# imagemagick/ImageMagick

Measured on NVIDIA H100. Metric: Mpixels/s on 8K RGBA Gaussian-blur σ=4 + Lanczos 2×; % HBM roofline, higher is better.
Workload: dtype f64

## Files before the change

imagemagick_b200/build.py:

```python
from __future__ import annotations

import os
import shutil
import subprocess
import sys
from concurrent.futures import ThreadPoolExecutor
from pathlib import Path

PKG = Path(__file__).resolve().parent
ROOT = PKG.parent
CSRC = PKG / "csrc"
LIBDIR = PKG / "lib"
OBJDIR = LIBDIR / "obj"
LIB = LIBDIR / "libmagickb200.so"

ARCH = ["-gencode", "arch=compute_90a,code=sm_90a"]
NVCC_FLAGS = ["-O3", "-std=c++17", "-lineinfo", "-Xcompiler", "-fPIC,-fvisibility=hidden,-ffp-contract=off",
              "-Xptxas", "-v"]

SOURCES = ["runtime.cu", "kernel_info.cpp", "resize_filter.cpp", "resize_tables.cpp", "conv1d.cu", "conv_mma.cu",
           "morph2d.cu", "morph_stream.cu", "morph_direct.cu", "cache.cu", "resize.cu", "resize_stream.cu", "colorspace.cu", "hexcone.cu", "pointwise.cu", "equalize.cu", "stencils.cu", "hooks.cu", "enhance.cu", "layout.cu", "level.cu",
           "distort_plan.cpp", "distort.cu", "geometry_plan.cpp", "geometry.cu", "api.cu"]
FILE_FLAGS = {"distort.cu": ["-fmad=false"]}


def _nvcc() -> str:
    for cand in (os.environ.get("NVCC"), shutil.which("nvcc"), "/usr/local/cuda/bin/nvcc"):
        if cand and Path(cand).exists():
            return cand
    raise RuntimeError("nvcc not found; libmagickb200 cannot be built")


def _stale(target: Path, deps: list[Path]) -> bool:
    if not target.exists():
        return True
    t = target.stat().st_mtime
    return any(d.stat().st_mtime > t for d in deps if d.exists())


def build(force: bool = False, verbose: bool = False) -> Path:
    nvcc = _nvcc()
    OBJDIR.mkdir(parents=True, exist_ok=True)
    headers = list(CSRC.glob("*.h")) + list(CSRC.glob("*.cuh")) + list((ROOT / "include").glob("*.h"))
    jobs = []
    for name in SOURCES:
        src = CSRC / name
        obj = OBJDIR / (src.stem + ".o")
        if force or _stale(obj, [src] + headers):
            cmd = [nvcc, *ARCH, *NVCC_FLAGS, *FILE_FLAGS.get(name, []), "-x", "cu", "-c", str(src), "-o", str(obj)]
            jobs.append((name, cmd, obj))

    def run(job):
        name, cmd, obj = job
        p = subprocess.run(cmd, capture_output=True, text=True)
# ... 27 lines not shown
```

imagemagick_b200/csrc/api.cu:

```cuda
#include "mb200_internal.h"

#include <cuda_runtime.h>

#include <cmath>
#include <cstdlib>
#include <memory>
#include <vector>

using namespace mb200;

namespace {

struct StreamAlloc {
  void *ptr = nullptr;
  cudaStream_t s;
  explicit StreamAlloc(cudaStream_t stream) : s(stream) {}
  int alloc(size_t bytes) {
    cudaError_t e = cudaMallocAsync(&ptr, bytes ? bytes : 1, temp_pool(), s);
    if (e != cudaSuccess) { ptr = nullptr; return cuda_fail(e, "cudaMallocAsync"); }
    return MB200_OK;
  }
  ~StreamAlloc() { if (ptr) cudaFreeAsync(ptr, s); }
  StreamAlloc(const StreamAlloc &) = delete;
  StreamAlloc &operator=(const StreamAlloc &) = delete;
// ... 80 lines not shown
          if (rc != MB200_EUNSUPPORTED) return rc;
        }
      }
    }
  }
  if ((method == MB200_ErodeMorphology || method == MB200_DilateMorphology) && d_counter == nullptr &&
      !knobs.no_morph_stream) {
    const int rc = launch_morph_stream(src, dst, w, h, ch, method, win.data(), kw, kh, ox, oy, s);
    if (rc != MB200_EUNSUPPORTED) return rc;
  }
  double gamma_scale = 1.0;
  if (method == MB200_ConvolveMorphology && kw == 1) {
    size_t count = 0;
    for (double v : win) if (!std::isnan(v)) ++count;
    if (count != 0) gamma_scale = static_cast<double>(kh) / static_cast<double>(count);
  }
  return launch_morph2d(src, dst, w, h, ch, method, win.data(), kw, kh, ox, oy, bias, gamma_scale, d_counter, s);
}

int counted_primitive(const float *src, float *dst, size_t w, size_t h, int ch, int method, const mb200_kernel_info *k,
                      double bias, unsigned long long *d_counter, long long *changed, cudaStream_t s) {
  cudaMemsetAsync(d_counter, 0, sizeof(unsigned long long), s);
  const int rc = primitive(src, dst, w, h, ch, method, k, bias, d_counter, s);
  if (rc) return rc;
  unsigned long long hostv = 0;
  cudaError_t e = cudaMemcpyAsync(&hostv, d_counter, sizeof(hostv), cudaMemcpyDeviceToHost, s);
  if (e == cudaSuccess) e = cudaStreamSynchronize(s);
  if (e != cudaSuccess) return cuda_fail(e, "changed readback");
  *changed = static_cast<long long>(hostv / static_cast<unsigned long long>(ch));
  return MB200_OK;
}

struct Stage { int primitive; const mb200_kernel_info *kernel; };

int apply_hit_and_miss_family(const float *src, float *dst, size_t w, size_t h, int ch, int method, long iterations,
                              const mb200_kernel_info *kernel, cudaStream_t s) {
  const size_t method_limit = iterations < 0 ? (w > h ? w : h) : static_cast<size_t>(iterations);
  const bool unite = method == MB200_HitAndMissMorphology && kernel->next != nullptr;
  const size_t bytes = w * h * static_cast<size_t>(ch) * sizeof(float), npix = w * h;
  StreamAlloc a(s), b(s), united(s), counter(s);
  int rc = a.alloc(bytes);
  if (!rc) rc = b.alloc(bytes);
  if (!rc && unite) rc = united.alloc(bytes);
  if (!rc) rc = counter.alloc(sizeof(unsigned long long));
  if (rc) return rc;
  float *bufs[2] = {static_cast<float *>(a.ptr), static_cast<float *>(b.ptr)};
  unsigned long long *d_counter = static_cast<unsigned long long *>(counter.ptr);
  const float *cur = src;
  int next = 0;
  bool have_united = false;
  size_t round = 0;
  long long round_changed = 1;
  while (round < method_limit && round_changed > 0) {
    ++round;
    round_changed = 0;
    for (const mb200_kernel_info *k = kernel; k; k = k->next) {
      if (method_limit > 1) {
        long long changed = 0;
        rc = counted_primitive(cur, bufs[next], w, h, ch, method, k, 0.0, d_counter, &changed, s);
        round_changed += changed;
      } else {
        rc = primitive(cur, bufs[next], w, h, ch, method, k, 0.0, nullptr, s);
      }
      if (rc) return rc;
      cur = bufs[next];
      next ^= 1;
// ... 63 lines not shown
    rotate_kernel_info(reflected.get(), 180.0);
  }
  std::vector<Stage> stages;
  const mb200_kernel_info *rk = reflected.get();
  for (const mb200_kernel_info *nk = kernel; nk; nk = nk->next, rk = rk ? rk->next : nullptr) {
    for (int stage = 1; stage <= stage_limit; ++stage) {
      Stage st{method, nk};
      switch (method) {
        case MB200_OpenMorphology: st.primitive = stage == 2 ? MB200_DilateMorphology : MB200_ErodeMorphology; break;
        case MB200_CloseMorphology: st.kernel = rk; st.primitive = stage == 2 ? MB200_ErodeMorphology : MB200_DilateMorphology; break;
        case MB200_OpenIntensityMorphology:
          st.primitive = stage == 2 ? MB200_DilateIntensityMorphology : MB200_ErodeIntensityMorphology;
          break;
        case MB200_CloseIntensityMorphology:
          st.kernel = rk;
          st.primitive = stage == 2 ? MB200_ErodeIntensityMorphology : MB200_DilateIntensityMorphology;
          break;
        case MB200_SmoothMorphology:
          if (stage == 1) st.primitive = MB200_ErodeMorphology;
          else if (stage == 2) st.primitive = MB200_DilateMorphology;
          else if (stage == 3) { st.kernel = rk; st.primitive = MB200_DilateMorphology; }
          else { st.kernel = rk; st.primitive = MB200_ErodeMorphology; }
          break;
        case MB200_CorrelateMorphology: st.kernel = rk; st.primitive = MB200_ConvolveMorphology; break;
        default: break;
      }
      stages.push_back(st);
    }
  }
  const size_t bytes = w * h * static_cast<size_t>(ch) * sizeof(float);
  int rc = MB200_OK;
  if (kernel_limit == 1) {
    const size_t total = stages.size();
    StreamAlloc tmp(s);
    if (total > 1) { rc = tmp.alloc(bytes); }
    const float *cur = src;
    for (size_t i = 0; i < total && rc == MB200_OK; ++i) {
      float *out = ((total - 1 - i) % 2 == 0) ? dst : static_cast<float *>(tmp.ptr);
      const bool last = i + 1 == total;
      rc = primitive(cur, out, w, h, ch, stages[i].primitive, stages[i].kernel, bias, nullptr, s,
                     last ? epilogue : nullptr, last ? epilogue_fused : nullptr);
      cur = out;
    }
  } else {
    StreamAlloc a(s), b(s), counter(s);
    rc = a.alloc(bytes);
    if (!rc) rc = b.alloc(bytes);
    if (!rc) rc = counter.alloc(sizeof(unsigned long long));
    const float *cur = src;
    float *bufs[2] = {static_cast<float *>(a.ptr), static_cast<float *>(b.ptr)};
    int next = 0;
    for (size_t i = 0; i < stages.size() && rc == MB200_OK; ++i) {
      size_t loop = 0;
      long long changed = 1;
      while (loop < kernel_limit && changed > 0 && rc == MB200_OK) {
        ++loop;
        rc = counted_primitive(cur, bufs[next], w, h, ch, stages[i].primitive, stages[i].kernel, bias,
                               static_cast<unsigned long long *>(counter.ptr), &changed, s);
        cur = bufs[next];
        next ^= 1;
      }
    }
    if (rc == MB200_OK) {
      cudaError_t e = cudaMemcpyAsync(dst, cur, bytes, cudaMemcpyDeviceToDevice, s);
      if (e != cudaSuccess) rc = cuda_fail(e, "result copy");
    }
// ... 1103 lines not shown
```

imagemagick_b200/csrc/conv_common.cuh:

```cuda
#pragma once

#include <cuda_runtime.h>

namespace mb200 {
namespace {

constexpr double kQuantumScale = 1.0 / 65535.0;
constexpr double kEpsilon = 1.0e-12;

__device__ __forceinline__ bool nonfinite_bits(float v) { return (__float_as_uint(v) & 0x7f800000u) == 0x7f800000u; }
__device__ __forceinline__ bool nonfinite_bits(double v) {
  return (static_cast<unsigned>(__double2hiint(v)) & 0x7ff00000u) == 0x7ff00000u;
}

__device__ __forceinline__ double clamp_denominator(double den) {
  constexpr double kTiny = kEpsilon / kQuantumScale;
  const unsigned hi = static_cast<unsigned>(__double2hiint(den));
  const unsigned long long mag = (static_cast<unsigned long long>(hi & 0x7fffffffu) << 32) | static_cast<unsigned>(__double2loint(den));
  const unsigned long long tiny = static_cast<unsigned long long>(__double_as_longlong(kTiny));
  if (mag < tiny)
    den = __hiloint2double(static_cast<int>((hi & 0x80000000u) | static_cast<unsigned>(tiny >> 32)), static_cast<int>(tiny & 0xffffffffu));
  return den;
}

__device__ __forceinline__ float unsharp_point(float p, float blurred, double gain, double qthreshold) {
  const double d = __dsub_rn(static_cast<double>(p), static_cast<double>(blurred));
  if (fabs(__dmul_rn(2.0, d)) < qthreshold) return p;
  return static_cast<float>(__dadd_rn(static_cast<double>(p), __dmul_rn(gain, d)));
}

__device__ __forceinline__ double fast_reciprocal(double g) {
  double r0;
  asm("rcp.approx.ftz.f64 %0, %1;" : "=d"(r0) : "d"(g));
  const double e0 = fma(-g, r0, 1.0);
  const double r1 = fma(r0, e0, r0);
  const double e1 = fma(-g, r1, 1.0);
  return fma(r1, e1, r1);
}

__device__ __forceinline__ double shfl_double(double v, int lane) {
  int lo = __double2loint(v), hi = __double2hiint(v);
  lo = __shfl_sync(0xffffffffu, lo, lane);
  hi = __shfl_sync(0xffffffffu, hi, lane);
  return __hiloint2double(hi, lo);
}

}
}
```

imagemagick_b200/csrc/conv_mma.cu:

```cuda
#include "mb200_internal.h"
#include "conv_common.cuh"

#include <cuda_runtime.h>

#include <cstdint>

namespace mb200 {
namespace {

template <int NKS>
struct MmaTaps { double k[4 * NKS]; };

struct MmaArgs {
  const void *src;
  void *dst;
  int width, height;
  int off;
  int ntaps;
  int strip;
  const float *aux;
  double gain, qthreshold;
  int l2pf;
};

// ... 246 lines not shown
      ahead[0] = raw[0]; ahead[1] = raw[1];
      raw[0] = keep0; raw[1] = keep1;
    }
    output(prev, epi_prev, prev_valid);
    if (b > 0) outp += ostep;

    if (window_bad != 0) {
#pragma unroll
      for (int g = 0; g < 2; ++g) {
        double s0 = 0.0, s1 = 0.0, s2 = 0.0, s3 = 0.0;
        int u = 8 * sb + n8;
        if (u >= RR) u -= RR;
        for (int t = 0; t < a.ntaps; ++t) {
          const double *p = ring + static_cast<unsigned>(u) * kUStride + lane_px_off + g * kGroup;
          const double2 rg = *reinterpret_cast<const double2 *>(p);
          const double2 ba = *reinterpret_cast<const double2 *>(p + kBA);
          const double k = taps.k[t];
          s0 = fma(k, rg.x, s0); s1 = fma(k, rg.y, s1); s2 = fma(k, ba.x, s2); s3 = fma(k, ba.y, s3);
          if (++u == RR) u = 0;
        }
        acc[2 * g][0] = s0; acc[2 * g][1] = s1; acc[2 * g + 1][0] = s2; acc[2 * g + 1][1] = s3;
      }
    }
#pragma unroll
    for (int t = 0; t < 4; ++t) { prev[t][0] = acc[t][0]; prev[t][1] = acc[t][1]; }
    if (EPI) { epi_prev[0] = epi_cur[0]; epi_prev[1] = epi_cur[1]; }
    prev_valid = mvalid;
    st_slot = st_slot + 1 == NB ? 0 : st_slot + 1;
    if (++sb == NB) sb = 0;
  }
  output(prev, epi_prev, prev_valid);
}

template <int NKS>
struct WideTaps { double k[16 * NKS]; };

template <int NKS, int AXIS, int EPI>
__global__ void __launch_bounds__(128, 3) conv_mma_wide_kernel(const MmaArgs a, const WideTaps<NKS> taps) {
  static_assert(EPI == 0 || AXIS == 1, "the fused epilogue belongs to the final column pass");
  constexpr int NB = NKS + 1;
  constexpr int RR = 16 * NB;
  constexpr int PW = 36;
  constexpr int PL = 2 * RR + 8;
  constexpr int kWarpDoubles = AXIS == 1 ? RR * PW : 16 * PL;
  extern __shared__ __align__(16) double ring_all[];
  const int warp = threadIdx.x >> 5, lane = threadIdx.x & 31;
  double *ring = ring_all + warp * kWarpDoubles;
  const unsigned ring_s = static_cast<unsigned>(__cvta_generic_to_shared(ring));
  const int t4 = lane & 3, g8 = lane >> 2;

  int first, nout, limit, par0;
  if (AXIS == 1) {
    par0 = (blockIdx.x * 4 + warp) * 8;
    if (par0 >= a.width) return;
    first = blockIdx.y * a.strip;
    nout = min(a.strip, a.height - first);
    limit = a.height - 1;
  } else {
    par0 = (blockIdx.y * 4 + warp) * 8;
    if (par0 >= a.height) return;
    first = blockIdx.x * a.strip;
    nout = min(a.strip, a.width - first);
    limit = a.width - 1;
  }
  const int nblocks = (nout + 15) >> 4;
  const bool mma_l2pf = a.l2pf != 0;
  const size_t pitch = static_cast<size_t>(a.width) * 16;

// ... 10 lines not shown
    } else {
      const int line = lh + 4 * (i >> 1);
      lbase[i] = static_cast<const char *>(a.src) + static_cast<size_t>(min(par0 + line, a.height - 1)) * pitch;
      uoff[i] = lq + 8 * (i & 1);
      st_off[i] = static_cast<unsigned>(line * PL + 2 * uoff[i]);
    }
  }
  constexpr unsigned kBlockStride = AXIS == 1 ? 16 * PW : 32;
  constexpr unsigned kBA = AXIS == 1 ? 16 : 8 * PL;
  const size_t lstep = AXIS == 1 ? pitch : 16;
  const int base = first - a.off;

  float4 raw[4];
  auto fetch = [&](int j) {
#pragma unroll
    for (int i = 0; i < 4; ++i) {
      const unsigned pos = static_cast<unsigned>(min(max(base + 16 * j + uoff[i], 0), limit));
      raw[i] = __ldg(reinterpret_cast<const float4 *>(lbase[i] + static_cast<size_t>(pos) * lstep));
    }
  };
  constexpr int kL2Ahead = 4;
  auto prefetch_l2 = [&](int j) {
#pragma unroll
    for (int i = 0; i < 4; ++i) {
      const unsigned pos = static_cast<unsigned>(min(max(base + 16 * j + uoff[i], 0), limit));
      asm volatile("prefetch.global.L2 [%0];" ::"l"(lbase[i] + static_cast<size_t>(pos) * lstep));
    }
  };
  unsigned badmask = 0;
  auto stage = [&](int slot) {
    bool bad = false;
#pragma unroll
    for (int i = 0; i < 4; ++i) {
      const float4 f = raw[i];
      const unsigned m = max(max(__float_as_uint(f.x) & 0x7fffffffu, __float_as_uint(f.y) & 0x7fffffffu),
                             max(__float_as_uint(f.z) & 0x7fffffffu, __float_as_uint(f.w) & 0x7fffffffu));
      bad = bad || m >= 0x7f800000u;
      const double da = static_cast<double>(f.w);
      double *q = ring + st_off[i] + static_cast<unsigned>(slot) * kBlockStride;
      *reinterpret_cast<double2 *>(q) = make_double2(static_cast<double>(f.x) * da, static_cast<double>(f.y) * da);
      *reinterpret_cast<double2 *>(q + kBA) = make_double2(static_cast<double>(f.z) * da, da);
    }
    const bool any = __any_sync(0xffffffffu, bad);
    badmask = any ? (badmask | (1u << slot)) : (badmask & ~(1u << slot));
  };

  constexpr int NA = 4 * NKS + 2;
  double atap[NA];
#pragma unroll
  for (int c = 0; c < NA; ++c) {
    const int t = 4 * (c - 2) + t4 - g8;
    const double v = taps.k[min(max(t, 0), 16 * NKS - 1)];
    atap[c] = (t >= 0 && t < a.ntaps) ? v : 0.0;
  }

  const unsigned frag_off = AXIS == 1 ? static_cast<unsigned>(t4 * PW + g8)
                                      : static_cast<unsigned>(2 * t4 + (g8 >> 1) * PL + (g8 & 1));
  constexpr unsigned kUStride = AXIS == 1 ? PW : 2;
  constexpr unsigned kT2 = AXIS == 1 ? 8 : 4 * PL;
  constexpr unsigned kTile[4] = {0, kBA, kT2, kT2 + kBA};
  const unsigned lane_px_off = AXIS == 1 ? static_cast<unsigned>(2 * t4) : static_cast<unsigned>(t4 * PL);

  char *outp;
  if (AXIS == 1) {
    outp = static_cast<char *>(a.dst) + static_cast<size_t>(first + g8) * pitch + static_cast<size_t>(par0 + t4) * 16;
  } else {
    outp = static_cast<char *>(a.dst) + static_cast<size_t>(par0 + t4) * pitch + static_cast<size_t>(first + g8) * 16;
  }
  const size_t ostep = AXIS == 1 ? 16 * pitch : 16 * 16;
  const size_t gstep = AXIS == 1 ? 4 * 16 : 4 * pitch;
  const size_t hstep = AXIS == 1 ? 8 * pitch : 8 * 16;
  bool gvalid[2];
#pragma unroll
  for (int g = 0; g < 2; ++g) gvalid[g] = (par0 + 4 * g + t4) < (AXIS == 1 ? a.width : a.height);
  auto output = [&](const double (&acc)[4][4], const float4 (&epi)[2][2], int mrem) {
#pragma unroll
    for (int g = 0; g < 2; ++g)
#pragma unroll
      for (int h = 0; h < 2; ++h) {
        const double sr = acc[2 * g][2 * h], sg = acc[2 * g][2 * h + 1], sbv = acc[2 * g + 1][2 * h],
                     sa = acc[2 * g + 1][2 * h + 1];
        const double r = fast_reciprocal(clamp_denominator(sa));
        float4 out = make_float4(static_cast<float>(sr * r), static_cast<float>(sg * r), static_cast<float>(sbv * r),
                                 static_cast<float>(sa));
        if (EPI) {
          out.x = unsharp_point(epi[g][h].x, out.x, a.gain, a.qthreshold);
          out.y = unsharp_point(epi[g][h].y, out.y, a.gain, a.qthreshold);
          out.z = unsharp_point(epi[g][h].z, out.z, a.gain, a.qthreshold);
          out.w = unsharp_point(epi[g][h].w, out.w, a.gain, a.qthreshold);
        }
        if (g8 + 8 * h < mrem && gvalid[g]) *reinterpret_cast<float4 *>(outp + g * gstep + h * hstep) = out;
      }
  };

  {
    float4 pre[NKS][4];
#pragma unroll
    for (int j = 0; j < NKS; ++j) {
      fetch(j);
#pragma unroll
      for (int i = 0; i < 4; ++i) pre[j][i] = raw[i];
    }
#pragma unroll
    for (int j = 0; j < NKS; ++j) {
#pragma unroll
      for (int i = 0; i < 4; ++i) raw[i] = pre[j][i];
      stage(j);
    }
  }
  float4 ahead[4];
  fetch(NKS + 1);
#pragma unroll
  for (int i = 0; i < 4; ++i) ahead[i] = raw[i];
  fetch(NKS);

  int st_slot = NKS, sb = 0;
  double prev[4][4];
#pragma unroll
  for (int t = 0; t < 4; ++t)
#pragma unroll
    for (int i = 0; i < 4; ++i) prev[t][i] = (i & 1) ? 1.0 : 0.0;
  float4 epi_prev[2][2], epi_cur[2][2];
#pragma unroll
// ... 12 lines not shown
    if (EPI) {
      const char *epip = reinterpret_cast<const char *>(a.aux) + (outp - static_cast<char *>(a.dst));
#pragma unroll
      for (int g = 0; g < 2; ++g)
#pragma unroll
        for (int h = 0; h < 2; ++h)
          if (g8 + 8 * h < mrem && gvalid[g])
            epi_cur[g][h] = __ldg(reinterpret_cast<const float4 *>(epip + g * gstep + h * hstep));
    }
    stage(st_slot);
#pragma unroll
    for (int i = 0; i < 4; ++i) raw[i] = ahead[i];
    {
      float4 keep[4];
#pragma unroll
      for (int i = 0; i < 4; ++i) keep[i] = raw[i];
      fetch(b + NKS + 2);
      if (mma_l2pf) prefetch_l2(b + NKS + 2 + kL2Ahead);
#pragma unroll
      for (int i = 0; i < 4; ++i) { ahead[i] = raw[i]; raw[i] = keep[i]; }
    }
    double acc[4][4];
#pragma unroll
    for (int t = 0; t < 4; ++t)
#pragma unroll
      for (int i = 0; i < 4; ++i) acc[t][i] = 0.0;
    {
      unsigned ua[NKS];
#pragma unroll
      for (int s = 0; s < NKS; ++s) {
        const int blk = sb + s >= NB ? sb + s - NB : sb + s;
        ua[s] = ring_s + (frag_off + static_cast<unsigned>(blk) * kBlockStride) * 8u;
      }
      auto lds4 = [&](double (&bv)[4], int q) {
        const unsigned addr = ua[q >> 2] + kTile[q & 3] * 8;
#pragma unroll
        for (int i = 0; i < 4; ++i)
          asm volatile("ld.shared.f64 %0, [%1];" : "=d"(bv[i]) : "r"(addr + 4 * i * kUStride * 8));
      };
      double bq[2][4];
      lds4(bq[0], 0);
#pragma unroll
      for (int q = 0; q < 4 * NKS; ++q) {
        if (q + 1 < 4 * NKS) lds4(bq[(q + 1) & 1], q + 1);
        const double *av = atap + 4 * (q >> 2);
        double (&d)[4] = acc[q & 3];
        const double (&bv)[4] = bq[q & 1];
        asm volatile("mma.sync.aligned.m16n8k16.row.col.f64.f64.f64.f64 {%0,%1,%2,%3}, {%4,%5,%6,%7,%8,%9,%10,%11}, "
                     "{%12,%13,%14,%15}, {%0,%1,%2,%3};"
                     : "+d"(d[0]), "+d"(d[1]), "+d"(d[2]), "+d"(d[3])
                     : "d"(av[2]), "d"(av[0]), "d"(av[3]), "d"(av[1]), "d"(av[4]), "d"(av[2]), "d"(av[5]), "d"(av[3]),
                       "d"(bv[0]), "d"(bv[1]), "d"(bv[2]), "d"(bv[3]));
      }
    }
    if (window_bad != 0) {
#pragma unroll
      for (int g = 0; g < 2; ++g)
#pragma unroll
        for (int h = 0; h < 2; ++h) {
          double s0 = 0.0, s1 = 0.0, s2 = 0.0, s3 = 0.0;
          int u = 16 * sb + g8 + 8 * h;
          if (u >= RR) u -= RR;
          for (int t = 0; t < a.ntaps; ++t) {
            const double *p = ring + static_cast<unsigned>(u) * kUStride + lane_px_off + g * kT2;
            const double2 rg = *reinterpret_cast<const double2 *>(p);
            const double2 ba = *reinterpret_cast<const double2 *>(p + kBA);
            const double k = taps.k[t];
            s0 = fma(k, rg.x, s0); s1 = fma(k, rg.y, s1); s2 = fma(k, ba.x, s2); s3 = fma(k, ba.y, s3);
            if (++u == RR) u = 0;
          }
          acc[2 * g][2 * h] = s0; acc[2 * g][2 * h + 1] = s1; acc[2 * g + 1][2 * h] = s2; acc[2 * g + 1][2 * h + 1] = s3;
        }
    }
#pragma unroll
    for (int t = 0; t < 4; ++t)
#pragma unroll
      for (int i = 0; i < 4; ++i) prev[t][i] = acc[t][i];
    if (EPI) {
#pragma unroll
      for (int g = 0; g < 2; ++g)
#pragma unroll
        for (int h = 0; h < 2; ++h) epi_prev[g][h] = epi_cur[g][h];
    }
    prev_rem = mrem;
    st_slot = st_slot + 1 == NB ? 0 : st_slot + 1;
    if (++sb == NB) sb = 0;
// ... 104 lines not shown
```

imagemagick_b200/csrc/mb200_internal.h:

```cpp
#pragma once

#include "../../include/magick_b200.h"

#include <cstddef>
#include <cstdint>
#include <memory>

struct CUmemPoolHandle_st;

extern "C" int mb200_resize_nearest(int filter, size_t in_n, size_t out_n, double factor, long *nearest);

namespace mb200 {

int fail(int code, const char *fmt, ...);
int cuda_fail(int cuda_error, const char *what);
void count_launch(unsigned n = 1);

struct TuningKnobs {
  int mma_strip, mma_minb, mma_l2pf, conv_mma, mma_wide;
  int pair, pair_async, pair_async_col, col_rot, row_pair_rot, row_rot;
  int resize_tma, resize_chunk, resize_slots, resize_strip;
  int no_rank1, no_morph_stream, no_resize_stream, resize_regular_h, no_fused_unsharp;
  int resize_fused, no_resize_fused;
  int conv2d_rows;
};
TuningKnobs tuning_knobs();

enum LaunchFamily {
  kConvMma, kConvMmaWide,
  kConvPair, kConvPairAsync, kConvGeneric,
  kResizeVStream, kResizeHTma, kResizeHStream, kResizeFused,
  kResizeRegular, kResizeGather,
  kConv2dDenseR8, kConv2dDenseR4, kConv2dDenseR2, kMorph2d, kMinmax2d,
  kMorphStream,
  kMorphDirect,
  kDistort,
  kGeometry,
  kLaunchFamilies
};
void count_family(LaunchFamily family);

struct DeviceState;
int ensure_device();
void *default_stream();
int scratch(void **ptr, size_t bytes, int slot);
int sm_count();
size_t l2_bytes();
::CUmemPoolHandle_st *temp_pool();

int copy_h2d(void *dev, const void *host, size_t bytes, void *stream);
int copy_d2h(void *host, const void *dev, size_t bytes, void *stream);
struct StageRef {
  void *entry = nullptr;
  void *dev = nullptr;
  void *host = nullptr;
  size_t bytes = 0;
  bool temporary = false;
};
int stage_input(const void *host, size_t bytes, void *stream, StageRef *out);
int stage_output(void *host, size_t bytes, void *stream, StageRef *out);
int finish_output(StageRef *ref, void *stream);
void release_stage(StageRef *ref, void *stream);

void rotate_kernel_info(mb200_kernel_info *k, double angle);
struct KernelInfoFree {
  void operator()(mb200_kernel_info *k) const { mb200_destroy_kernel_info(k); }
};
using KernelList = std::unique_ptr<mb200_kernel_info, KernelInfoFree>;
KernelList blur_kernel_pair(double radius, double sigma);

inline bool has_alpha(int channels) { return channels == 2 || channels == 4; }


struct UnsharpEpilogue { const float *source; double gain, quantum_threshold; };
int launch_conv1d(const float *src, float *dst, size_t width, size_t height, int channels,
                  int axis, const double *taps_window_order, int ntaps, int origin_offset,
                  double bias, double gamma_scale, unsigned long long *d_changed, void *stream,
                  int io = 0,
                  const UnsharpEpilogue *epilogue = nullptr, bool *epilogue_fused = nullptr);

int launch_conv_mma(const void *src, void *dst, size_t width, size_t height, int axis, const double *taps_window_order,
                    int ntaps, int origin_offset, void *stream, int io, const UnsharpEpilogue *epilogue,
                    bool *epilogue_fused);

int launch_morph2d(const float *src, float *dst, size_t width, size_t height, int channels,
                   int method, const double *kernel_window_order, int kw, int kh, int ox, int oy,
                   double bias, double gamma_scale, unsigned long long *d_changed, void *stream);

int launch_morph_stream(const float *src, float *dst, size_t width, size_t height, int channels, int method,
                        const double *kernel_window_order, int kw, int kh, int ox, int oy, void *stream);

int morphology_direct_check(int channels, int method, const mb200_kernel_info *kernel);
int launch_morphology_direct(const float *src, float *tmp, float *dst, size_t width, size_t height, int channels,
                             int method, const mb200_kernel_info *kernel, void *stream);

int distort_check(size_t width, size_t height, int channels, const mb200_distort_params *plan,
                  const mb200_resample_options *options);
int launch_distort(const float *src, size_t width, size_t height, int channels, float *dst,
                   const mb200_distort_params *plan, const mb200_resample_options *options, void *stream);

int geometry_check(size_t width, size_t height, int channels, const mb200_geometry_params *plan);
int launch_geometry(const float *src, size_t width, size_t height, int channels, float *dst,
                    const mb200_geometry_params *plan, void *stream);

#define MB200_RESIZE_MAX_SEGMENTS 8
struct ResizeAxis {
  int device = -1, filter = 0;
  mb200_filter_options options{};
  size_t in_n = 0, out_n = 0;
  long taps = 0;
  int max_span = 0, reg_stride = 0, reg_taps = 0;
  int *d_start = nullptr, *d_count = nullptr;
  double *d_weights = nullptr;
  double *d_wreg = nullptr;
  int nseg = 0, seg_o[MB200_RESIZE_MAX_SEGMENTS], seg_n[MB200_RESIZE_MAX_SEGMENTS], seg_src[MB200_RESIZE_MAX_SEGMENTS];
  double *d_wsets = nullptr;
// ... 95 lines not shown
```

imagemagick_b200/csrc/runtime.cu:

```cuda
#include "mb200_internal.h"

#include <cuda_runtime.h>

#include <atomic>
#include <cctype>
#include <climits>
#include <cstdarg>
#include <cstdio>
#include <cstdlib>
#include <cstring>
#include <mutex>

namespace mb200 {

namespace {
thread_local char t_error[512] = "";
std::atomic<unsigned long long> g_launches{0};

constexpr int kMaxDevices = 16;
constexpr int kScratchSlots = 8;

struct DeviceStateImpl {
  bool ready = false;
  cudaStream_t stream = nullptr;
// ... 16 lines not shown
}

int cuda_fail(int e, const char *what) {
  const cudaError_t err = static_cast<cudaError_t>(e);
  if (err == cudaErrorNoDevice || err == cudaErrorInsufficientDriver)
    return fail(MB200_ENODEVICE, "%s: %s", what, cudaGetErrorString(err));
  if (err == cudaErrorMemoryAllocation) return fail(MB200_ENOMEM, "%s: %s", what, cudaGetErrorString(err));
  return fail(MB200_ECUDA, "%s: %s", what, cudaGetErrorString(err));
}

void count_launch(unsigned n) { g_launches.fetch_add(n, std::memory_order_relaxed); }

namespace {
constexpr int kKnobMax = 1 << 20;
enum KnobKind {
  kInteger,
  kSwitch,
};
struct KnobSpec {
  const char *name;
  int TuningKnobs::*field;
  int fallback;
  bool (*valid)(int);
  KnobKind kind;
  const char *env;
};
bool any_value(int) { return true; }
const KnobSpec kKnobs[] = {
    {"mma_strip", &TuningKnobs::mma_strip, 512, [](int v) { return v >= 8 && v <= kKnobMax; }},
    {"mma_minb", &TuningKnobs::mma_minb, 4, [](int v) { return v == 3 || v == 4; }},
    {"mma_l2pf", &TuningKnobs::mma_l2pf, -1, [](int v) { return v >= -1 && v <= 1; }},
    {"conv_mma", &TuningKnobs::conv_mma, -1, [](int v) { return v >= -1 && v <= 1; }, kInteger, "MB200_MMA"},
    {"mma_wide", &TuningKnobs::mma_wide, -1, [](int v) { return v >= -1 && v <= 1; }},
    {"pair", &TuningKnobs::pair, 1, [](int v) { return v == 0 || v == 1; }},
    {"pair_async", &TuningKnobs::pair_async, 1, [](int v) { return v == 0 || v == 1; }},
    {"pair_async_col", &TuningKnobs::pair_async_col, -1, [](int v) { return v >= -1 && v <= 1; }},
    {"col_rot", &TuningKnobs::col_rot, 16, [](int v) { return v >= 1 && v <= kKnobMax; }},
    {"row_pair_rot", &TuningKnobs::row_pair_rot, 16, [](int v) { return v >= 1 && v <= kKnobMax; }},
    {"row_rot", &TuningKnobs::row_rot, 0, [](int v) { return v >= 0 && v <= kKnobMax; }},
    {"resize_tma", &TuningKnobs::resize_tma, 1, [](int v) { return v >= 0 && v <= 2; }},
    {"resize_chunk", &TuningKnobs::resize_chunk, 16, [](int v) { return v == 8 || v == 16; }},
    {"resize_slots", &TuningKnobs::resize_slots, 0, [](int v) { return v == 0 || v == 2 || v == 3; }},
    {"resize_strip", &TuningKnobs::resize_strip, 0, [](int v) { return v >= 0 && v <= kKnobMax; }},
    {"conv2d_rows", &TuningKnobs::conv2d_rows, 0, [](int v) { return v == 0 || v == 2 || v == 4 || v == 8; }},
    {"no_rank1", &TuningKnobs::no_rank1, 0, any_value, kSwitch},
    {"no_morph_stream", &TuningKnobs::no_morph_stream, 0, any_value, kSwitch},
    {"no_resize_stream", &TuningKnobs::no_resize_stream, 0, any_value, kSwitch},
    {"no_fused_unsharp", &TuningKnobs::no_fused_unsharp, 0, any_value, kSwitch},
    {"no_resize_fused", &TuningKnobs::no_resize_fused, 0, any_value, kSwitch},
    {"resize_regular_h", &TuningKnobs::resize_regular_h, 0, any_value, kSwitch},
    {"resize_fused", &TuningKnobs::resize_fused, 0, any_value, kSwitch},
};
constexpr size_t kNumKnobs = sizeof(kKnobs) / sizeof(kKnobs[0]);

int parse_env(const KnobSpec &k, const char *s) {
  if (!s || !*s) return k.fallback;
  if (k.kind == kSwitch) return *s != '0';
  char *end = nullptr;
  const long parsed = std::strtol(s, &end, 10);
  if (*end == '\0' && parsed >= INT_MIN && parsed <= INT_MAX && k.valid(static_cast<int>(parsed)))
    return static_cast<int>(parsed);
  return k.fallback;
}

struct KnobStore {
  std::atomic<int> value[kNumKnobs];
  KnobStore() {
    for (size_t i = 0; i < kNumKnobs; ++i) {
      char env[64] = "MB200_";
      for (size_t j = 0; kKnobs[i].name[j] && j + 7 < sizeof(env); ++j)
        env[6 + j] = static_cast<char>(std::toupper(static_cast<unsigned char>(kKnobs[i].name[j])));
      value[i].store(parse_env(kKnobs[i], std::getenv(kKnobs[i].env ? kKnobs[i].env : env)), std::memory_order_relaxed);
    }
  }
};
KnobStore &knob_store() {
  static KnobStore s;
  return s;
}
int knob_index(const char *name) {
  for (size_t i = 0; i < kNumKnobs; ++i)
    if (std::strcmp(kKnobs[i].name, name) == 0) return static_cast<int>(i);
  return -1;
}

const char *const kFamilyNames[kLaunchFamilies] = {
    "conv_mma_launches", "conv_mma_wide_launches", "conv_pair_launches", "conv_pair_async_launches", "conv_generic_launches",
    "resize_v_stream_launches", "resize_h_tma_launches", "resize_h_stream_launches", "resize_fused_launches",
    "resize_regular_launches", "resize_gather_launches", "conv2d_dense_r8_launches", "conv2d_dense_r4_launches",
    "conv2d_dense_r2_launches", "morph2d_launches", "minmax2d_launches", "morph_stream_launches", "morph_direct_launches",
    "distort_launches", "geometry_launches"};
std::atomic<unsigned long long> g_family_launches[kLaunchFamilies];
int family_index(const char *name) {
  for (int f = 0; f < kLaunchFamilies; ++f)
    if (std::strcmp(kFamilyNames[f], name) == 0) return f;
  return -1;
}
}

TuningKnobs tuning_knobs() {
  TuningKnobs t;
  KnobStore &s = knob_store();
  for (size_t i = 0; i < kNumKnobs; ++i) t.*kKnobs[i].field = s.value[i].load(std::memory_order_relaxed);
  return t;
}

void count_family(LaunchFamily family) { g_family_launches[family].fetch_add(1, std::memory_order_relaxed); }

int ensure_device() {
  int dev = -1;
  cudaError_t e = cudaGetDevice(&dev);
  if (e != cudaSuccess) { cudaGetLastError(); return cuda_fail(e, "cudaGetDevice"); }
  if (dev < 0 || dev >= kMaxDevices) return fail(MB200_ENODEVICE, "device index %d out of range", dev);
  std::lock_guard<std::mutex> lock(g_mutex);
  DeviceStateImpl &d = g_dev[dev];
  if (d.ready) return MB200_OK;
  cudaDeviceProp prop;
  e = cudaGetDeviceProperties(&prop, dev);
  if (e != cudaSuccess) return cuda_fail(e, "cudaGetDeviceProperties");
  if (prop.major != 9 || prop.minor != 0)
// ... 236 lines not shown
```

Before: 26670.

## Fuse separable Gaussian row and column passes into one tensor-core kernel

Adds a fused kernel that runs the horizontal FP64 MMA convolution into a shared-memory ring buffer, then runs the vertical MMA pass from that ring within the same block. This removes the intermediate full-image write and read between the two separable passes, cutting HBM traffic. It applies only to 4-channel, zero-bias kernels of 18 to 33 taps, and by default only when the image exceeds L2. In exchange it recomputes row halos per strip and uses more shared memory, which limits occupancy to two blocks per SM.

New measurement: 28200, median of 6. 1.06x the previous value.

```diff
diff --git a/imagemagick_b200/build.py b/imagemagick_b200/build.py
--- a/imagemagick_b200/build.py
+++ b/imagemagick_b200/build.py
@@ -19,7 +19,7 @@
               "-Xptxas", "-v"]
 
 SOURCES = ["runtime.cu", "kernel_info.cpp", "resize_filter.cpp", "resize_tables.cpp", "conv1d.cu", "conv_mma.cu",
-           "morph2d.cu", "morph_stream.cu", "morph_direct.cu", "cache.cu", "resize.cu", "resize_stream.cu", "colorspace.cu", "hexcone.cu", "pointwise.cu", "equalize.cu", "stencils.cu", "hooks.cu", "enhance.cu", "layout.cu", "level.cu",
+           "conv_fused.cu", "morph2d.cu", "morph_stream.cu", "morph_direct.cu", "cache.cu", "resize.cu", "resize_stream.cu", "colorspace.cu", "hexcone.cu", "pointwise.cu", "equalize.cu", "stencils.cu", "hooks.cu", "enhance.cu", "layout.cu", "level.cu",
            "distort_plan.cpp", "distort.cu", "geometry_plan.cpp", "geometry.cu", "api.cu"]
 FILE_FLAGS = {"distort.cu": ["-fmad=false"]}
 
diff --git a/imagemagick_b200/csrc/api.cu b/imagemagick_b200/csrc/api.cu
--- a/imagemagick_b200/csrc/api.cu
+++ b/imagemagick_b200/csrc/api.cu
@@ -136,6 +136,23 @@
 }
 
 struct Stage { int primitive; const mb200_kernel_info *kernel; };
+
+int fused_blur(const float *src, float *dst, size_t w, size_t h, const Stage &row, const Stage &col,
+               const UnsharpEpilogue *epilogue, bool *epilogue_fused, cudaStream_t s) {
+  if (row.primitive != MB200_ConvolveMorphology || col.primitive != MB200_ConvolveMorphology) return MB200_EUNSUPPORTED;
+  const mb200_kernel_info *rk = row.kernel, *ck = col.kernel;
+  if (rk->height != 1 || rk->width < 18 || rk->width > 33 || ck->width != 1 || ck->height < 18 || ck->height > 33 ||
+      rk->y != 0 || ck->x != 0)
+    return MB200_EUNSUPPORTED;
+  double rt[33], ct[33];
+  const int rn = static_cast<int>(rk->width), cn = static_cast<int>(ck->height);
+  for (int i = 0; i < rn; ++i) rt[i] = rk->values[rn - 1 - i];
+  for (int i = 0; i < cn; ++i) ct[i] = ck->values[cn - 1 - i];
+  for (int i = 0; i < rn; ++i) if (std::isnan(rt[i])) return MB200_EUNSUPPORTED;
+  for (int i = 0; i < cn; ++i) if (std::isnan(ct[i])) return MB200_EUNSUPPORTED;
+  const int ox = rn - static_cast<int>(rk->x) - 1, oy = cn - static_cast<int>(ck->y) - 1;
+  return launch_conv_mma_fused_blur(src, dst, w, h, rt, rn, ox, ct, cn, oy, epilogue, epilogue_fused, s);
+}
 
 int apply_hit_and_miss_family(const float *src, float *dst, size_t w, size_t h, int ch, int method, long iterations,
                               const mb200_kernel_info *kernel, cudaStream_t s) {
@@ -265,6 +282,11 @@
   int rc = MB200_OK;
   if (kernel_limit == 1) {
     const size_t total = stages.size();
+    if (total == 2 && ch == 4 && bias == 0.0) {
+      rc = fused_blur(src, dst, w, h, stages[0], stages[1], epilogue, epilogue_fused, s);
+      if (rc != MB200_EUNSUPPORTED) return rc;
+      rc = MB200_OK;
+    }
     StreamAlloc tmp(s);
     if (total > 1) { rc = tmp.alloc(bytes); }
     const float *cur = src;
diff --git a/imagemagick_b200/csrc/conv_common.cuh b/imagemagick_b200/csrc/conv_common.cuh
--- a/imagemagick_b200/csrc/conv_common.cuh
+++ b/imagemagick_b200/csrc/conv_common.cuh
@@ -38,6 +38,63 @@
   return fma(r1, e1, r1);
 }
 
+__device__ __forceinline__ bool nonfinite4(float4 f) {
+  const unsigned m = max(max(__float_as_uint(f.x) & 0x7fffffffu, __float_as_uint(f.y) & 0x7fffffffu),
+                         max(__float_as_uint(f.z) & 0x7fffffffu, __float_as_uint(f.w) & 0x7fffffffu));
+  return m >= 0x7f800000u;
+}
+__device__ __forceinline__ void premultiply(float4 f, double2 &rg, double2 &ba) {
+  const double da = static_cast<double>(f.w);
+  rg = make_double2(static_cast<double>(f.x) * da, static_cast<double>(f.y) * da);
+  ba = make_double2(static_cast<double>(f.z) * da, da);
+}
+__device__ __forceinline__ float4 normalise_sums(double sr, double sg, double sb, double sa) {
+  const double r = fast_reciprocal(clamp_denominator(sa));
+  return make_float4(static_cast<float>(sr * r), static_cast<float>(sg * r), static_cast<float>(sb * r),
+                     static_cast<float>(sa));
+}
+__device__ __forceinline__ float4 unsharp_point4(float4 p, float4 blurred, double gain, double qthreshold) {
+  return make_float4(unsharp_point(p.x, blurred.x, gain, qthreshold), unsharp_point(p.y, blurred.y, gain, qthreshold),
+                     unsharp_point(p.z, blurred.z, gain, qthreshold), unsharp_point(p.w, blurred.w, gain, qthreshold));
+}
+
+template <int NKS>
+struct WideTaps { double k[16 * NKS]; };
+
+template <int NKS>
+__device__ __forceinline__ void wide_tap_fragments(double (&atap)[4 * NKS + 2], const WideTaps<NKS> &taps, int ntaps,
+                                                   int lane) {
+  const int t4 = lane & 3, g8 = lane >> 2;
+#pragma unroll
+  for (int c = 0; c < 4 * NKS + 2; ++c) {
+    const int t = 4 * (c - 2) + t4 - g8;
+    const double v = taps.k[min(max(t, 0), 16 * NKS - 1)];
+    atap[c] = (t >= 0 && t < ntaps) ? v : 0.0;
+  }
+}
+
+template <int NKS, typename Addr>
+__device__ __forceinline__ void wide_mma(double (&acc)[4][4], const double (&atap)[4 * NKS + 2], Addr addr) {
+  auto lds4 = [&](double (&bv)[4], int q) {
+#pragma unroll
+    for (int i = 0; i < 4; ++i) asm volatile("ld.shared.f64 %0, [%1];" : "=d"(bv[i]) : "r"(addr(q, i)));
+  };
+  double bq[2][4];
+  lds4(bq[0], 0);
+#pragma unroll
+  for (int q = 0; q < 4 * NKS; ++q) {
+    if (q + 1 < 4 * NKS) lds4(bq[(q + 1) & 1], q + 1);
+    const double *av = atap + 4 * (q >> 2);
+    double (&d)[4] = acc[q & 3];
+    const double (&bv)[4] = bq[q & 1];
+    asm volatile("mma.sync.aligned.m16n8k16.row.col.f64.f64.f64.f64 {%0,%1,%2,%3}, {%4,%5,%6,%7,%8,%9,%10,%11}, "
+                 "{%12,%13,%14,%15}, {%0,%1,%2,%3};"
+                 : "+d"(d[0]), "+d"(d[1]), "+d"(d[2]), "+d"(d[3])
+                 : "d"(av[2]), "d"(av[0]), "d"(av[3]), "d"(av[1]), "d"(av[4]), "d"(av[2]), "d"(av[5]), "d"(av[3]),
+                   "d"(bv[0]), "d"(bv[1]), "d"(bv[2]), "d"(bv[3]));
+  }
+}
+
 __device__ __forceinline__ double shfl_double(double v, int lane) {
   int lo = __double2loint(v), hi = __double2hiint(v);
   lo = __shfl_sync(0xffffffffu, lo, lane);
diff --git a/imagemagick_b200/csrc/conv_fused.cu b/imagemagick_b200/csrc/conv_fused.cu
--- /dev/null
+++ b/imagemagick_b200/csrc/conv_fused.cu
@@ -0,0 +1,285 @@
+#include "mb200_internal.h"
+#include "conv_common.cuh"
+
+#include <cuda_runtime.h>
+
+#include <cstdint>
+
+namespace mb200 {
+namespace {
+
+constexpr int kNKS = 3;
+constexpr int kWt = 32;
+constexpr int kPL = 2 * 64 + 8;
+constexpr int kLineGroup = 16 * kPL;
+constexpr int kPW = 36;
+constexpr int kRingRows = 64;
+constexpr int kColGroup = kRingRows * kPW;
+constexpr size_t kSmemBytes = (2 * kLineGroup + 4 * kColGroup) * sizeof(double) + 4 * sizeof(unsigned long long) +
+                              8 * sizeof(int);
+
+struct FusedArgs {
+  const float4 *src;
+  float4 *dst;
+  int width, height;
+  int roff, rntaps;
+  int coff, cntaps;
+  int strip;
+  const float4 *aux;
+  double gain, qthreshold;
+};
+
+template <int EPI>
+__global__ void __launch_bounds__(128, 2)
+conv_mma_fused_blur_kernel(const FusedArgs a, const WideTaps<kNKS> rtaps, const WideTaps<kNKS> ctaps) {
+  extern __shared__ __align__(16) double smem[];
+  double *stg = smem;
+  double *cring = smem + 2 * kLineGroup;
+  unsigned long long *colbad = reinterpret_cast<unsigned long long *>(cring + 4 * kColGroup);
+  int *rowbad = reinterpret_cast<int *>(colbad + 4);
+  const unsigned stg_s = static_cast<unsigned>(__cvta_generic_to_shared(stg));
+  const unsigned cring_s = static_cast<unsigned>(__cvta_generic_to_shared(cring));
+  const int warp = threadIdx.x >> 5, lane = threadIdx.x & 31;
+  const int t4 = lane & 3, g8 = lane >> 2;
+  const int W = a.width, H = a.height;
+  const int x0 = blockIdx.x * kWt, y0 = blockIdx.y * a.strip;
+  const int nout = min(a.strip, H - y0);
+  const int nb = (nout + 15) >> 4;
+
+  double ratap[4 * kNKS + 2], catap[4 * kNKS + 2];
+  wide_tap_fragments<kNKS>(ratap, rtaps, a.rntaps, lane);
+  wide_tap_fragments<kNKS>(catap, ctaps, a.cntaps, lane);
+
+  const int lg = warp >> 1, rh = warp & 1;
+  const int lq = lane & 7, lh = lane >> 3;
+  int colx[4];
+  unsigned st_off[4];
+#pragma unroll
+  for (int c = 0; c < 4; ++c) {
+    const int pos = 16 * (2 * rh + (c >> 1)) + lq + 8 * (c & 1);
+    colx[c] = min(max(x0 - a.roff + pos, 0), W - 1);
+    st_off[c] = static_cast<unsigned>(lg * kLineGroup + lh * kPL + 2 * pos);
+  }
+  float4 raw[8];
+  auto fetch = [&](int blk) {
+#pragma unroll
+    for (int j = 0; j < 2; ++j) {
+      const int y = min(16 * blk + 8 * lg + lh + 4 * j, H - 1);
+      const float4 *line = a.src + static_cast<size_t>(y) * W;
+#pragma unroll
+      for (int c = 0; c < 4; ++c) raw[4 * j + c] = __ldg(line + colx[c]);
+    }
+  };
+  auto stage = [&]() {
+    bool bad[2] = {false, false};
+#pragma unroll
+    for (int j = 0; j < 2; ++j)
+#pragma unroll
+      for (int c = 0; c < 4; ++c) {
+        const float4 f = raw[4 * j + c];
+        bad[c >> 1] = bad[c >> 1] || nonfinite4(f);
+        double2 rg, ba;
+        premultiply(f, rg, ba);
+        double *q = stg + st_off[c] + 4 * j * kPL;
+        *reinterpret_cast<double2 *>(q) = rg;
+        *reinterpret_cast<double2 *>(q + 8 * kPL) = ba;
+      }
+    const bool b0 = __any_sync(0xffffffffu, bad[0]), b1 = __any_sync(0xffffffffu, bad[1]);
+    if (lane == 0) { rowbad[4 * lg + 2 * rh] = b0; rowbad[4 * lg + 2 * rh + 1] = b1; }
+  };
+  const unsigned rfrag = stg_s + static_cast<unsigned>(lg * kLineGroup + 2 * t4 + (g8 >> 1) * kPL + (g8 & 1)) * 8u +
+                         static_cast<unsigned>(32 * rh) * 8u;
+  constexpr unsigned kRowTile[4] = {0, 8 * kPL, 4 * kPL, 12 * kPL};
+
+  auto row_phase = [&](int blk) {
+    double acc[4][4];
+#pragma unroll
+    for (int t = 0; t < 4; ++t)
+#pragma unroll
+      for (int i = 0; i < 4; ++i) acc[t][i] = 0.0;
+    wide_mma<kNKS>(acc, ratap, [&](int q, int i) { return rfrag + (32 * (q >> 2) + kRowTile[q & 3] + 8 * i) * 8u; });
+    if ((rowbad[4 * lg + rh] | rowbad[4 * lg + rh + 1] | rowbad[4 * lg + rh + 2]) != 0) {
+#pragma unroll
+      for (int g = 0; g < 2; ++g)
+#pragma unroll
+        for (int h = 0; h < 2; ++h) {
+          double s0 = 0.0, s1 = 0.0, s2 = 0.0, s3 = 0.0;
+          const double *p = stg + lg * kLineGroup + 2 * (16 * rh + g8 + 8 * h) + (4 * g + t4) * kPL;
+          for (int t = 0; t < a.rntaps; ++t) {
+            const double2 rg = *reinterpret_cast<const double2 *>(p + 2 * t);
+            const double2 ba = *reinterpret_cast<const double2 *>(p + 2 * t + 8 * kPL);
+            const double k = rtaps.k[t];
+            s0 = fma(k, rg.x, s0); s1 = fma(k, rg.y, s1); s2 = fma(k, ba.x, s2); s3 = fma(k, ba.y, s3);
+          }
+          acc[2 * g][2 * h] = s0; acc[2 * g][2 * h + 1] = s1; acc[2 * g + 1][2 * h] = s2; acc[2 * g + 1][2 * h + 1] = s3;
+        }
+    }
+    const int rrow = 16 * (blk & 3) + 8 * lg;
+    unsigned char flags[2] = {0, 0};
+#pragma unroll
+    for (int h = 0; h < 2; ++h) {
+      const bool inside = x0 + 16 * rh + g8 + 8 * h < W;
+#pragma unroll
+      for (int g = 0; g < 2; ++g) {
+        const float4 f = normalise_sums(acc[2 * g][2 * h], acc[2 * g][2 * h + 1], acc[2 * g + 1][2 * h],
+                                        acc[2 * g + 1][2 * h + 1]);
+        unsigned bits = __ballot_sync(0xffffffffu, inside && nonfinite4(f));
+        bits |= bits >> 16; bits |= bits >> 8; bits |= bits >> 4;
+        flags[h] |= static_cast<unsigned char>((bits & 0xfu) << (4 * g));
+        double2 rg, ba;
+        premultiply(f, rg, ba);
+        double *q = cring + (2 * rh + h) * kColGroup + (rrow + 4 * g + t4) * kPW + 2 * g8;
+        *reinterpret_cast<double2 *>(q) = rg;
+        *reinterpret_cast<double2 *>(q + 16) = ba;
+      }
+    }
+    if (lane == 0) {
+#pragma unroll
+      for (int h = 0; h < 2; ++h)
+        reinterpret_cast<unsigned char *>(colbad + 2 * rh + h)[2 * (blk & 3) + lg] = flags[h];
+    }
+  };
+
+  const int par0 = x0 + 8 * warp;
+  const bool col_active = par0 < W;
+  bool gvalid[2];
+#pragma unroll
+  for (int g = 0; g < 2; ++g) gvalid[g] = par0 + 4 * g + t4 < W;
+  const unsigned cgroup_s = cring_s + static_cast<unsigned>(warp * kColGroup + g8) * 8u;
+  constexpr unsigned kColTile[4] = {0, 16, 8, 24};
+  const double *cgroup = cring + warp * kColGroup;
+
+  auto col_phase = [&](int b) {
+    const int yb = y0 + 16 * b;
+    const int ya = yb - a.coff;
+    const int mrem = nout - 16 * b;
+    float4 epi[2][2];
+    const size_t obase = static_cast<size_t>(yb + g8) * W + par0 + t4;
+    if (EPI) {
+#pragma unroll
+      for (int g = 0; g < 2; ++g)
+#pragma unroll
+        for (int h = 0; h < 2; ++h)
+          epi[g][h] = (g8 + 8 * h < mrem && gvalid[g]) ? __ldg(a.aux + obase + static_cast<size_t>(8 * h) * W + 4 * g)
+                                                       : make_float4(0.f, 0.f, 0.f, 0.f);
+    }
+    unsigned rowaddr[kNKS][4];
+#pragma unroll
+    for (int s = 0; s < kNKS; ++s)
+#pragma unroll
+      for (int i = 0; i < 4; ++i) {
+        const int y = min(max(ya + 16 * s + t4 + 4 * i, 0), H - 1);
+        rowaddr[s][i] = cgroup_s + static_cast<unsigned>((y & (kRingRows - 1)) * kPW) * 8u;
+      }
+    double acc[4][4];
+#pragma unroll
+    for (int t = 0; t < 4; ++t)
+#pragma unroll
+      for (int i = 0; i < 4; ++i) acc[t][i] = 0.0;
+    wide_mma<kNKS>(acc, catap, [&](int q, int i) { return rowaddr[q >> 2][i] + kColTile[q & 3] * 8u; });
+    const int clo = min(max(ya, 0), H - 1), chi = min(max(ya + 16 * kNKS - 1, 0), H - 1);
+    const unsigned long long m = colbad[warp];
+    const int rot = clo & (kRingRows - 1);
+    const unsigned long long rotated = rot ? (m >> rot) | (m << (kRingRows - rot)) : m;
+    if ((rotated & ((1ull << (chi - clo + 1)) - 1)) != 0) {
+#pragma unroll
+      for (int g = 0; g < 2; ++g)
+#pragma unroll
+        for (int h = 0; h < 2; ++h) {
+          double s0 = 0.0, s1 = 0.0, s2 = 0.0, s3 = 0.0;
+          for (int t = 0; t < a.cntaps; ++t) {
+            const int y = min(max(ya + g8 + 8 * h + t, 0), H - 1);
+            const double *p = cgroup + (y & (kRingRows - 1)) * kPW + 2 * t4 + 8 * g;
+            const double2 rg = *reinterpret_cast<const double2 *>(p);
+            const double2 ba = *reinterpret_cast<const double2 *>(p + 16);
+            const double k = ctaps.k[t];
+            s0 = fma(k, rg.x, s0); s1 = fma(k, rg.y, s1); s2 = fma(k, ba.x, s2); s3 = fma(k, ba.y, s3);
+          }
+          acc[2 * g][2 * h] = s0; acc[2 * g][2 * h + 1] = s1; acc[2 * g + 1][2 * h] = s2; acc[2 * g + 1][2 * h + 1] = s3;
+        }
+    }
+#pragma unroll
+    for (int g = 0; g < 2; ++g)
+#pragma unroll
+      for (int h = 0; h < 2; ++h) {
+        float4 out = normalise_sums(acc[2 * g][2 * h], acc[2 * g][2 * h + 1], acc[2 * g + 1][2 * h],
+                                    acc[2 * g + 1][2 * h + 1]);
+        if (EPI) out = unsharp_point4(epi[g][h], out, a.gain, a.qthreshold);
+        if (g8 + 8 * h < mrem && gvalid[g]) a.dst[obase + static_cast<size_t>(8 * h) * W + 4 * g] = out;
+      }
+  };
+
+  auto blk_of = [&](int y) { return min(max(y, 0), H - 1) >> 4; };
+  int next = blk_of(y0 - a.coff);
+  const int last = blk_of(y0 + 16 * (nb - 1) - a.coff + 16 * kNKS - 1);
+  fetch(next);
+#pragma unroll 1
+  for (int b = 0; b < nb; ++b) {
+    const int hi = blk_of(y0 + 16 * b - a.coff + 16 * kNKS - 1);
+#pragma unroll 1
+    for (; next <= hi; ++next) {
+      stage();
+      if (next < last) fetch(next + 1);
+      __syncthreads();
+      row_phase(next);
+      __syncthreads();
+    }
+    if (col_active) col_phase(b);
+  }
+}
+
+template <int EPI>
+void launch_epi(const FusedArgs &a, const WideTaps<kNKS> &rt, const WideTaps<kNKS> &ct, dim3 grid, cudaStream_t s) {
+  auto kernel = conv_mma_fused_blur_kernel<EPI>;
+  cudaFuncSetAttribute(kernel, cudaFuncAttributeMaxDynamicSharedMemorySize, static_cast<int>(kSmemBytes));
+  kernel<<<grid, 128, kSmemBytes, s>>>(a, rt, ct);
+}
+
+}
+
+int launch_conv_mma_fused_blur(const float *src, float *dst, size_t width, size_t height, const double *row_taps,
+                               int row_ntaps, int row_offset, const double *col_taps, int col_ntaps, int col_offset,
+                               const UnsharpEpilogue *epilogue, bool *epilogue_fused, void *stream) {
+  if (epilogue_fused) *epilogue_fused = false;
+  const TuningKnobs knobs = tuning_knobs();
+  if (knobs.blur_fused == 0 || knobs.conv_mma == 0 || knobs.mma_wide == 0) return MB200_EUNSUPPORTED;
+  if (row_ntaps < 18 || row_ntaps > 33 || col_ntaps < 18 || col_ntaps > 33) return MB200_EUNSUPPORTED;
+  if (row_offset < 0 || row_offset >= row_ntaps || col_offset < 0 || col_offset >= col_ntaps) return MB200_EUNSUPPORTED;
+  if (width == 0 || height == 0 || width * 32 > 0x7fffffffull || height > 0x3fffffffull) return MB200_EUNSUPPORTED;
+  if (((reinterpret_cast<uintptr_t>(src) | reinterpret_cast<uintptr_t>(dst)) & 15) != 0) return MB200_EUNSUPPORTED;
+  const size_t bytes = width * height * 16;
+  const uintptr_t s0 = reinterpret_cast<uintptr_t>(src), d0 = reinterpret_cast<uintptr_t>(dst);
+  if (s0 < d0 + bytes && d0 < s0 + bytes) return MB200_EUNSUPPORTED;
+  if (knobs.blur_fused < 0 && bytes <= l2_bytes()) return MB200_EUNSUPPORTED;
+  const int strip = (knobs.mma_strip + 15) & ~15;
+  if ((height + 31) / 32 > 65535 || (height + strip - 1) / strip > 65535) return MB200_EUNSUPPORTED;
+  FusedArgs a{};
+  a.src = reinterpret_cast<const float4 *>(src);
+  a.dst = reinterpret_cast<float4 *>(dst);
+  a.width = static_cast<int>(width); a.height = static_cast<int>(height);
+  a.roff = row_offset; a.rntaps = row_ntaps;
+  a.coff = col_offset; a.cntaps = col_ntaps;
+  a.strip = strip;
+  const bool epi = epilogue && epilogue->source && (reinterpret_cast<uintptr_t>(epilogue->source) & 15) == 0;
+  if (epi) {
+    a.aux = reinterpret_cast<const float4 *>(epilogue->source);
+    a.gain = epilogue->gain; a.qthreshold = epilogue->quantum_threshold;
+  }
+  WideTaps<kNKS> rt, ct;
+  for (int i = 0; i < 16 * kNKS; ++i) {
+    rt.k[i] = i < row_ntaps ? row_taps[i] : 0.0;
+    ct.k[i] = i < col_ntaps ? col_taps[i] : 0.0;
+  }
+  const dim3 grid(static_cast<unsigned>((width + kWt - 1) / kWt), static_cast<unsigned>((height + strip - 1) / strip));
+  cudaStream_t s = static_cast<cudaStream_t>(stream);
+  if (epi) launch_epi<1>(a, rt, ct, grid, s);
+  else launch_epi<0>(a, rt, ct, grid, s);
+  count_launch();
+  count_family(kConvMmaFused);
+  const cudaError_t e = cudaGetLastError();
+  if (e != cudaSuccess) return cuda_fail(e, "conv_mma_fused_blur launch");
+  if (epilogue_fused) *epilogue_fused = epi;
+  return MB200_OK;
+}
+
+}
diff --git a/imagemagick_b200/csrc/conv_mma.cu b/imagemagick_b200/csrc/conv_mma.cu
--- a/imagemagick_b200/csrc/conv_mma.cu
+++ b/imagemagick_b200/csrc/conv_mma.cu
@@ -302,8 +302,6 @@
   output(prev, epi_prev, prev_valid);
 }
 
-template <int NKS>
-struct WideTaps { double k[16 * NKS]; };
 
 template <int NKS, int AXIS, int EPI>
 __global__ void __launch_bounds__(128, 3) conv_mma_wide_kernel(const MmaArgs a, const WideTaps<NKS> taps) {
@@ -380,27 +378,19 @@
     bool bad = false;
 #pragma unroll
     for (int i = 0; i < 4; ++i) {
-      const float4 f = raw[i];
-      const unsigned m = max(max(__float_as_uint(f.x) & 0x7fffffffu, __float_as_uint(f.y) & 0x7fffffffu),
-                             max(__float_as_uint(f.z) & 0x7fffffffu, __float_as_uint(f.w) & 0x7fffffffu));
-      bad = bad || m >= 0x7f800000u;
-      const double da = static_cast<double>(f.w);
+      bad = bad || nonfinite4(raw[i]);
+      double2 rg, ba;
+      premultiply(raw[i], rg, ba);
       double *q = ring + st_off[i] + static_cast<unsigned>(slot) * kBlockStride;
-      *reinterpret_cast<double2 *>(q) = make_double2(static_cast<double>(f.x) * da, static_cast<double>(f.y) * da);
-      *reinterpret_cast<double2 *>(q + kBA) = make_double2(static_cast<double>(f.z) * da, da);
+      *reinterpret_cast<double2 *>(q) = rg;
+      *reinterpret_cast<double2 *>(q + kBA) = ba;
     }
     const bool any = __any_sync(0xffffffffu, bad);
     badmask = any ? (badmask | (1u << slot)) : (badmask & ~(1u << slot));
   };
 
-  constexpr int NA = 4 * NKS + 2;
-  double atap[NA];
-#pragma unroll
-  for (int c = 0; c < NA; ++c) {
-    const int t = 4 * (c - 2) + t4 - g8;
-    const double v = taps.k[min(max(t, 0), 16 * NKS - 1)];
-    atap[c] = (t >= 0 && t < a.ntaps) ? v : 0.0;
-  }
+  double atap[4 * NKS + 2];
+  wide_tap_fragments<NKS>(atap, taps, a.ntaps, lane);
 
   const unsigned frag_off = AXIS == 1 ? static_cast<unsigned>(t4 * PW + g8)
                                       : static_cast<unsigned>(2 * t4 + (g8 >> 1) * PL + (g8 & 1));
@@ -426,17 +416,9 @@
     for (int g = 0; g < 2; ++g)
 #pragma unroll
       for (int h = 0; h < 2; ++h) {
-        const double sr = acc[2 * g][2 * h], sg = acc[2 * g][2 * h + 1], sbv = acc[2 * g + 1][2 * h],
-                     sa = acc[2 * g + 1][2 * h + 1];
-        const double r = fast_reciprocal(clamp_denominator(sa));
-        float4 out = make_float4(static_cast<float>(sr * r), static_cast<float>(sg * r), static_cast<float>(sbv * r),
-                                 static_cast<float>(sa));
-        if (EPI) {
-          out.x = unsharp_point(epi[g][h].x, out.x, a.gain, a.qthreshold);
-          out.y = unsharp_point(epi[g][h].y, out.y, a.gain, a.qthreshold);
-          out.z = unsharp_point(epi[g][h].z, out.z, a.gain, a.qthreshold);
-          out.w = unsharp_point(epi[g][h].w, out.w, a.gain, a.qthreshold);
-        }
+        float4 out = normalise_sums(acc[2 * g][2 * h], acc[2 * g][2 * h + 1], acc[2 * g + 1][2 * h],
+                                    acc[2 * g + 1][2 * h + 1]);
+        if (EPI) out = unsharp_point4(epi[g][h], out, a.gain, a.qthreshold);
         if (g8 + 8 * h < mrem && gvalid[g]) *reinterpret_cast<float4 *>(outp + g * gstep + h * hstep) = out;
       }
   };
@@ -515,26 +497,7 @@
         const int blk = sb + s >= NB ? sb + s - NB : sb + s;
         ua[s] = ring_s + (frag_off + static_cast<unsigned>(blk) * kBlockStride) * 8u;
       }
-      auto lds4 = [&](double (&bv)[4], int q) {
-        const unsigned addr = ua[q >> 2] + kTile[q & 3] * 8;
-#pragma unroll
-        for (int i = 0; i < 4; ++i)
-          asm volatile("ld.shared.f64 %0, [%1];" : "=d"(bv[i]) : "r"(addr + 4 * i * kUStride * 8));
-      };
-      double bq[2][4];
-      lds4(bq[0], 0);
-#pragma unroll
-      for (int q = 0; q < 4 * NKS; ++q) {
-        if (q + 1 < 4 * NKS) lds4(bq[(q + 1) & 1], q + 1);
-        const double *av = atap + 4 * (q >> 2);
-        double (&d)[4] = acc[q & 3];
-        const double (&bv)[4] = bq[q & 1];
-        asm volatile("mma.sync.aligned.m16n8k16.row.col.f64.f64.f64.f64 {%0,%1,%2,%3}, {%4,%5,%6,%7,%8,%9,%10,%11}, "
-                     "{%12,%13,%14,%15}, {%0,%1,%2,%3};"
-                     : "+d"(d[0]), "+d"(d[1]), "+d"(d[2]), "+d"(d[3])
-                     : "d"(av[2]), "d"(av[0]), "d"(av[3]), "d"(av[1]), "d"(av[4]), "d"(av[2]), "d"(av[5]), "d"(av[3]),
-                       "d"(bv[0]), "d"(bv[1]), "d"(bv[2]), "d"(bv[3]));
-      }
+      wide_mma<NKS>(acc, atap, [&](int q, int i) { return ua[q >> 2] + kTile[q & 3] * 8 + 4 * i * kUStride * 8; });
     }
     if (window_bad != 0) {
 #pragma unroll
diff --git a/imagemagick_b200/csrc/mb200_internal.h b/imagemagick_b200/csrc/mb200_internal.h
--- a/imagemagick_b200/csrc/mb200_internal.h
+++ b/imagemagick_b200/csrc/mb200_internal.h
@@ -23,11 +23,13 @@
   int no_rank1, no_morph_stream, no_resize_stream, resize_regular_h, no_fused_unsharp;
   int resize_fused, no_resize_fused;
   int conv2d_rows;
+  int blur_fused;
 };
 TuningKnobs tuning_knobs();
 
 enum LaunchFamily {
   kConvMma, kConvMmaWide,
+  kConvMmaFused,
   kConvPair, kConvPairAsync, kConvGeneric,
   kResizeVStream, kResizeHTma, kResizeHStream, kResizeFused,
   kResizeRegular, kResizeGather,
@@ -82,6 +84,10 @@
 int launch_conv_mma(const void *src, void *dst, size_t width, size_t height, int axis, const double *taps_window_order,
                     int ntaps, int origin_offset, void *stream, int io, const UnsharpEpilogue *epilogue,
                     bool *epilogue_fused);
+
+int launch_conv_mma_fused_blur(const float *src, float *dst, size_t width, size_t height, const double *row_taps,
+                               int row_ntaps, int row_offset, const double *col_taps, int col_ntaps, int col_offset,
+                               const UnsharpEpilogue *epilogue, bool *epilogue_fused, void *stream);
 
 int launch_morph2d(const float *src, float *dst, size_t width, size_t height, int channels,
                    int method, const double *kernel_window_order, int kw, int kh, int ox, int oy,
diff --git a/imagemagick_b200/csrc/runtime.cu b/imagemagick_b200/csrc/runtime.cu
--- a/imagemagick_b200/csrc/runtime.cu
+++ b/imagemagick_b200/csrc/runtime.cu
@@ -72,6 +72,7 @@
     {"mma_l2pf", &TuningKnobs::mma_l2pf, -1, [](int v) { return v >= -1 && v <= 1; }},
     {"conv_mma", &TuningKnobs::conv_mma, -1, [](int v) { return v >= -1 && v <= 1; }, kInteger, "MB200_MMA"},
     {"mma_wide", &TuningKnobs::mma_wide, -1, [](int v) { return v >= -1 && v <= 1; }},
+    {"blur_fused", &TuningKnobs::blur_fused, -1, [](int v) { return v >= -1 && v <= 1; }},
     {"pair", &TuningKnobs::pair, 1, [](int v) { return v == 0 || v == 1; }},
     {"pair_async", &TuningKnobs::pair_async, 1, [](int v) { return v == 0 || v == 1; }},
     {"pair_async_col", &TuningKnobs::pair_async_col, -1, [](int v) { return v >= -1 && v <= 1; }},
@@ -125,7 +126,7 @@
 }
 
 const char *const kFamilyNames[kLaunchFamilies] = {
-    "conv_mma_launches", "conv_mma_wide_launches", "conv_pair_launches", "conv_pair_async_launches", "conv_generic_launches",
+    "conv_mma_launches", "conv_mma_wide_launches", "conv_mma_fused_launches", "conv_pair_launches", "conv_pair_async_launches", "conv_generic_launches",
     "resize_v_stream_launches", "resize_h_tma_launches", "resize_h_stream_launches", "resize_fused_launches",
     "resize_regular_launches", "resize_gather_launches", "conv2d_dense_r8_launches", "conv2d_dense_r4_launches",
     "conv2d_dense_r2_launches", "morph2d_launches", "minmax2d_launches", "morph_stream_launches", "morph_direct_launches",
```
